# JoeMWatson/input-inference-for-control

Measured on AMD Instinct MI355X. Metric: i2c timestep-messages/sec (cell-iterations/s = B*T*EM-iters/s), pendulum T=200 B=4096 per GPU, higher is better.
Workload: dtype f64; 1 GPU; pendulum_known_quad cubature i2c (nx=2, nu=1, nz=4), T=200, B=4096 trajectories per GPU, global batch 4096, CubatureQuadrature(1,0,0), alpha0=100, tol=0; batch_per_gpu=4096, horizon=200, parallelism=batch-sharded x1, no collective in the EM loop, kernels=one lane per trajectory

## Files before the change

### input-inference-for-control_amd/csrc/i2c_cell.hpp

```cpp
#pragma once
#include <stdint.h>
#include <type_traits>
#include "../../include/i2c_hip.h"
#include "i2c_linalg.hpp"
#include "i2c_models.hpp"

namespace i2c {

template <typename R> struct Rule {
  R sf;
  R w0;
  R wi;
  R W;
  int unit;
  int gh_degree, gh_points;
  R gh_x[I2C_MAX_GH_DEGREE], gh_w[I2C_MAX_GH_DEGREE];
};

template <class M> struct PerTraj : M {};
template <class M> struct is_per_traj : std::false_type {};
template <class M> struct is_per_traj<PerTraj<M>> : std::true_type {};
template <typename R, bool PER_TRAJ> struct ParamsB {};
template <typename R> struct ParamsB<R, true> {
  const R* params_b;
// ... 524 lines not shown
inline thread_local GridLaneSim grid_lane_sim{0, nullptr};
inline void grid_sim_sync();
#endif
I2C_FN int grid_lane() {
#ifdef I2C_HOST_SIM
  return grid_lane_sim.l;
#else
  return (int)__builtin_amdgcn_mbcnt_hi(~0u, __builtin_amdgcn_mbcnt_lo(~0u, 0u));
#endif
}
template <int GRID> I2C_FN bool grid_writer() {
  if constexpr (GRID == GRID_WAVE) return grid_lane() == 0;
  else return true;
}
template <int GRID> I2C_FN void grid_read_before_write() {
#ifdef I2C_HOST_SIM
  if constexpr (GRID == GRID_WAVE) grid_sim_sync();
#endif
}
template <class M, int DIN, int DOUT, bool CROSS, typename R, class F>
I2C_FN void grid_transform_wave(const Rule<R>& rule, const R* m, const R* L, const F& f, R* my, R* Sy, R* Sxy);

template <int GRID, class M, class ST, int DIN, int DOUT, bool CROSS, bool UNITW = false, typename R, class F>
I2C_FN void transform(const Rule<R>& rule, const R* m, const R* Sin, const R* L, const F& f, R* my, R* Sy, R* Sxy,
                      const PolyTab<R>* tab = nullptr) {
  if constexpr (GRID == GRID_WAVE) {
    grid_transform_wave<M, DIN, DOUT, CROSS>(rule, m, L, f, my, Sy, Sxy);
  } else if constexpr (GRID != 0) {
    if constexpr (DIN <= 3) {
      if (rule.gh_degree == 3) return grid_transform_ct<M, 3, DIN, DOUT, CROSS>(rule, m, L, f, my, Sy, Sxy);
      if (rule.gh_degree == 4) return grid_transform_ct<M, 4, DIN, DOUT, CROSS>(rule, m, L, f, my, Sy, Sxy);
      if (rule.gh_degree == 2) return grid_transform_ct<M, 2, DIN, DOUT, CROSS>(rule, m, L, f, my, Sy, Sxy);
    }
    grid_transform<M, DIN, DOUT, CROSS>(rule, m, L, f, my, Sy, Sxy);
  } else
    sp_transform<M, ST, DIN, DOUT, CROSS, UNITW>(rule, m, Sin, L, f, my, Sy, Sxy, tab);
}


template <typename R, typename S = R> struct FwdArgs {
  const S* prior;
  S* fwd;
  S* prior_out;
  const R* x0;
  const R* sig_x0;
  const R* z;
  const R* alpha;
  const R* alpha_cell;
  const uint8_t* ff;
  int32_t* status;
  const uint8_t* expert;
};

template <class M, typename R, bool LEAN = false, int GRID = 0, typename ST_ = R>
I2C_HD inline void forward_sweep_body(const Consts<M, R>& c, const FwdArgs<R, ST_>& a, const int b) {
  using C = Consts<M, R>;
  constexpr int NX = C::NX, NU = C::NU, NZ = C::NZ, NZT = C::NZT, D = C::D;
  constexpr unsigned W = sizeof(ST_);
  const unsigned long B = c.B;
  const int T = c.T;
  const unsigned bo = (unsigned)b * W;
  const unsigned rb0 = (unsigned)(B * W);
  const R alpha_traj = a.alpha[b];
  const bool wr = grid_writer<GRID>();
  int fail = 0;

  R mu_x[NX], sig_x[sym(NX)];
#pragma unroll
  for (int i = 0; i < NX; ++i) mu_x[i] = a.x0[i * B + b];
#pragma unroll
  for (int i = 0; i < sym(NX); ++i) sig_x[i] = a.sig_x0[i * B + b];

  constexpr bool VOFF = C::D <= 5;
  unsigned voff[VOFF ? C::E_FWD : 1];
  if (VOFF) {
#pragma unroll
    for (int e = 0; e < C::E_FWD; ++e) voff[e] = bo + (unsigned)e * rb0;
  }
  constexpr bool PREFETCH = C::D <= 5;
  R pri[C::E_PRI], zt[NZ];
  if (PREFETCH) {
    const unsigned rb = rb0;
    const Window w = make_window(a.prior + (unsigned long)(LEAN ? 0 : c.row(0)) * C::E_POST * B, (unsigned long)C::E_POST * rb);
#pragma unroll
    for (int e = 0; e < C::E_PRI; ++e) pri[e] = (R)wld<ST_>(w, VOFF ? 0u : (e) * rb, VOFF ? voff[e] : bo);
#pragma unroll
    for (int k = 0; k < NZ; ++k) zt[k] = (!LEAN && c.z_per_cell) ? a.z[((long)c.row(0) * NZ + k) * B + b] : c.zg[k];
  }

  unsigned ff_cur = a.ff[LEAN ? 0 : c.row(0)];
  constexpr bool STRUCT_L0 = C::D <= 5;
  R Lx[STRUCT_L0 ? sym(NX) : 1];
  if (STRUCT_L0) {
    R rx[NX];
#pragma unroll
    for (int i = 0; i < sym(NX); ++i) Lx[i] = sig_x[i];
    fail = note_failure(fail, chol<NX>(Lx, rx), 1, 0);
  }

  ff_cur = opaque(ff_cur);
  if (PREFETCH) {
#pragma unroll
    for (int e = 0; e < C::E_PRI; ++e) pri[e] = opaque(pri[e]);
#pragma unroll
    for (int k = 0; k < NZ; ++k) zt[k] = opaque(zt[k]);
  }
#pragma unroll
  for (int i = 0; i < NX; ++i) mu_x[i] = opaque(mu_x[i]);
#pragma unroll
  for (int i = 0; i < sym(NX); ++i) sig_x[i] = opaque(sig_x[i]);
  const R alpha_settled = opaque(alpha_traj);
  R alpha_cur = opaque((!LEAN && a.alpha_cell) ? a.alpha_cell[(long)c.row(0) * B + b] : alpha_settled);
  constexpr bool CONST_V = VOFF && (sym(NZ) + sym(NX) <= 16);
  PolyTab<R> ptab;
  if (CONST_V) poly_tab_init(ptab);
  const PolyTab<R>* const tab = CONST_V ? &ptab : nullptr;
  R xi0_v[CONST_V ? sym(NZ) : 1], eta_v[CONST_V ? sym(NX) : 1];
  if (CONST_V) {
#pragma unroll
    for (int i = 0; i < sym(NZ); ++i) xi0_v[i] = opaque(c.sig_xi0[i]);
#pragma unroll
    for (int i = 0; i < sym(NX); ++i) eta_v[i] = opaque(LEAN ? c.sig_eta[i] : c.sig_eta_w[i]);
  }

  for (int t = 0; t < T; ++t) {
    const int tn = t + 1 < T ? t + 1 : t;
    const int tr = LEAN ? t : c.row(t), tnr = LEAN ? tn : c.row(tn);
    const unsigned rb = opaque_uniform(rb0);
    const int kz = (C::D >= 6) ? (int)opaque_uniform(0u) : 0;
    if (!PREFETCH) {
      const Window w = make_window(a.prior + (unsigned long)tr * C::E_POST * B, (unsigned long)C::E_POST * rb);
#pragma unroll
      for (int e = 0; e < C::E_PRI; ++e) pri[e] = (R)wld<ST_>(w, VOFF ? 0u : (e) * rb, VOFF ? voff[e] : bo);
#pragma unroll
      for (int k = 0; k < NZ; ++k) zt[k] = (!LEAN && c.z_per_cell) ? a.z[((long)tr * NZ + k) * B + b] : c.zg[k];
    }

    const R alpha = opaque(alpha_cur);
    const R* pmu = pri;
    const R* psig = pri + D;
    const R* Kprev = pri + D + sym(D);

    int cell_bad = 0;
    R mu0[D], S0[sym(D)];
    R L0[STRUCT_L0 ? sym(D) : 1], Luu[sym(NU)], ruu[NU];
    if (ff_cur != 0) {
#pragma unroll
      for (int i = 0; i < NX; ++i) mu0[i] = mu_x[i];
#pragma unroll
      for (int i = NX; i < D; ++i) mu0[i] = pmu[i];
#pragma unroll
      for (int i = 0; i < D; ++i)
#pragma unroll
        for (int j = 0; j <= i; ++j)
          S0[tri(i, j)] = (i < NX) ? sig_x[tri(i, j)] : (j >= NX ? psig[tri(i, j)] : R(0));
      if (STRUCT_L0) {
#pragma unroll
        for (int p = 0; p < NU; ++p)
#pragma unroll
          for (int q = 0; q <= p; ++q) Luu[tri(p, q)] = psig[tri(NX + p, NX + q)];
#pragma unroll
        for (int p = 0; p < NU; ++p)
#pragma unroll
          for (int j = 0; j < NX; ++j) L0[tri(NX + p, j)] = R(0);
      }
    } else {
      R S[sym(NX)], delta[NX];
#pragma unroll
      for (int i = 0; i < sym(NX); ++i) S[i] = psig[i] + sig_x[i];
#pragma unroll
      for (int i = 0; i < NX; ++i) delta[i] = mu_x[i] - pmu[i];
      bool ok;
      const R rho = pdf_ratio<NX>(S, delta, &ok, tab);
      cell_bad = flag_stage(cell_bad, ok, 0);
      R Kt[NU * NX];
#pragma unroll
      for (int i = 0; i < NU * NX; ++i) Kt[i] = rho * Kprev[i];
// ... 59 lines not shown
      R mz[NZ], Sz[sym(NZ)], Sxz[D * NZ];
      transform<GRID, M, ObsStruct<M>, D, NZ, true, LEAN>(c.rule_xu, mu0, S0, L, ObserveF<M, R>{params_of(c, b)}, mz, Sz, Sxz, tab);
#pragma unroll
      for (int i = 0; i < sym(NZ); ++i) Sz[i] += alpha * (CONST_V ? xi0_v[i] : c.sig_xi0[i + kz]);
      cell_bad = flag_stage(cell_bad, kalman_update<D, NZ>(mu0, S0, mz, Sz, Sxz, zt), 2);
    }
    if (!LEAN && PREFETCH && c.z_per_cell) {
#pragma unroll
      for (int k = 0; k < NZ; ++k) zt[k] = a.z[((long)tnr * NZ + k) * B + b];
    }
    const Window out = make_window(a.fwd + (unsigned long)t * C::E_FWD * B, (unsigned long)C::E_FWD * rb);
    if (wr) {
#pragma unroll
      for (int e = 0; e < D; ++e) wst(out, VOFF ? 0u : (e) * rb, VOFF ? voff[e] : bo, (ST_)mu0[e]);
#pragma unroll
      for (int e = 0; e < sym(D); ++e) wst(out, VOFF ? 0u : (D + e) * rb, VOFF ? voff[D + e] : bo, (ST_)S0[e]);
    }

    sched_fence<(D >= 6)>();
    R Sxy[D * NX];
    {
      R L[sym(D)], rinv[D];
#pragma unroll
      for (int i = 0; i < sym(D); ++i) L[i] = S0[i];
      cell_bad = flag_stage(cell_bad, chol<D>(L, rinv), 3);
      transform<GRID, M, DenseStruct<D>, D, NX, true, LEAN>(c.rule_xu, mu0, S0, L, DynamicsF<M, R>{params_of(c, b)}, mu_x, sig_x, Sxy, tab);
    }
#pragma unroll
    for (int i = 0; i < sym(NX); ++i) sig_x[i] += CONST_V ? eta_v[i] : (LEAN ? c.sig_eta[i + kz] : c.sig_eta_w[i + kz]);
    R L3[sym(NX)], rinv3[NX];
#pragma unroll
    for (int i = 0; i < sym(NX); ++i) L3[i] = sig_x[i];
    cell_bad = flag_stage(cell_bad, chol<NX>(L3, rinv3), 4);
    sched_fence<(D >= 6)>();
#pragma unroll
    for (int i = 0; i < D; ++i) {
      fsub<NX>(L3, rinv3, &Sxy[i * NX]);
      bsub<NX>(L3, rinv3, &Sxy[i * NX]);
      sched_fence<(D >= 6)>();
    }

    ff_cur = opaque(ff_cur);
    if (!LEAN) {
      alpha_cur = opaque(alpha_cur);
      if (PREFETCH) {
#pragma unroll
        for (int k = 0; k < NZ; ++k) zt[k] = opaque(zt[k]);
      }
    }
    if (PREFETCH) {
#pragma unroll
      for (int e = 0; e < C::E_PRI; ++e) pri[e] = opaque(pri[e]);
    }
    if (wr) {
#pragma unroll
      for (int e = 0; e < D * NX; ++e) wst(out, VOFF ? 0u : (D + sym(D) + NX + sym(NX) + e) * rb, VOFF ? voff[D + sym(D) + NX + sym(NX) + e] : bo, (ST_)Sxy[e]);
    }
    sched_fence<(D >= 6)>();

    if (NZT > 0 && t == c.terminal_cell && c.has_Qf) {
      constexpr int NT = C::NZT1;
      R mzt[NT], Szt[sym(NT)], Sxzt[NX * NT];
      transform<GRID, M, TermStruct<M>, NX, NT, true, LEAN>(c.rule_x, mu_x, sig_x, L3, ObserveTermF<M, R>{params_of(c, b)}, mzt, Szt, Sxzt);
#pragma unroll
      for (int i = 0; i < sym(NT); ++i) Szt[i] += alpha * c.sig_xiT0[i];
      cell_bad = flag_stage(cell_bad, kalman_update<NX, NT>(mu_x, sig_x, mzt, Szt, Sxzt, c.zg_term), 5);
      if (STRUCT_L0) {
#pragma unroll
        for (int i = 0; i < sym(NX); ++i) L3[i] = sig_x[i];
        cell_bad = flag_stage(cell_bad, chol<NX>(L3, rinv3), 5);
      }
    }
    if (STRUCT_L0) {
#pragma unroll
      for (int i = 0; i < sym(NX); ++i) Lx[i] = L3[i];
    }
    fail = fold_cell_failure(fail, cell_bad, t);
    if (wr) {
#pragma unroll
      for (int e = 0; e < NX; ++e) wst(out, VOFF ? 0u : (D + sym(D) + e) * rb, VOFF ? voff[D + sym(D) + e] : bo, (ST_)mu_x[e]);
#pragma unroll
      for (int e = 0; e < sym(NX); ++e) wst(out, VOFF ? 0u : (D + sym(D) + NX + e) * rb, VOFF ? voff[D + sym(D) + NX + e] : bo, (ST_)sig_x[e]);
    }

  }
  if (wr && fail != 0 && a.status[b] == 0) a.status[b] = fail;
}


template <class M, typename R, int GRID = 0>
I2C_FN void end_of_chain(const Consts<M, R>& c, R* temp, const int b, const R* m3f, const R* S3f, R* m3m, R* S3m,
                         int32_t* status) {
  constexpr int NX = M::NX;
  const bool wr = grid_writer<GRID>();
  if (c.has_x_terminal) {
    const R tmp = temp[b];
    grid_read_before_write<GRID>();
    if (wr) temp[b] = tmp + c.dtemp;
    R St[sym(NX)], Ssum[sym(NX)], rinv[NX];
#pragma unroll
    for (int i = 0; i < sym(NX); ++i) {
      St[i] = tmp * S3f[i];
      Ssum[i] = c.sig_x_term[i] + St[i];
    }
    bool ok = chol<NX>(Ssum, rinv);
    R Wm[NX * NX];
#pragma unroll
    for (int j = 0; j < NX; ++j) {
      R col[NX];
#pragma unroll
      for (int i = 0; i < NX; ++i) col[i] = St[tri_any(i, j)];
      fsub<NX>(Ssum, rinv, col);
#pragma unroll
      for (int i = 0; i < NX; ++i) Wm[i * NX + j] = col[i];
    }
#pragma unroll
    for (int i = 0; i < NX; ++i)
#pragma unroll
      for (int j = 0; j <= i; ++j) {
        R v = St[tri(i, j)];
#pragma unroll
        for (int k = 0; k < NX; ++k) v -= Wm[k * NX + i] * Wm[k * NX + j];
        S3m[tri(i, j)] = v;
      }
    R r1[NX], r2[NX], Lt[sym(NX)], LT[sym(NX)];
#pragma unroll
    for (int i = 0; i < sym(NX); ++i) {
      Lt[i] = St[i];
      LT[i] = c.sig_x_term[i];
    }
    ok = chol<NX>(Lt, rinv) && ok;
#pragma unroll
    for (int i = 0; i < NX; ++i) r1[i] = m3f[i];
    fsub<NX>(Lt, rinv, r1);
    bsub<NX>(Lt, rinv, r1);
    ok = chol<NX>(LT, rinv) && ok;
#pragma unroll
    for (int i = 0; i < NX; ++i) r2[i] = c.mu_x_term[i];
// ... 1229 lines not shown
```

### input-inference-for-control_amd/csrc/i2c_impl.hpp

```cpp
#pragma once
#include "i2c_entry.hpp"
#include "i2c_cell.hpp"
#include "i2c_group.hpp"
#include "i2c_wave.hpp"
#include "i2c_quad.hpp"
#include "i2c_grid.hpp"
#include "i2c_linearize.hpp"

#include <cmath>
#include <cstdlib>
#include <cstring>

namespace i2c {

constexpr int SWEEP_BLOCK = 64;
#ifndef I2C_LANE_BLOCK
#define I2C_LANE_BLOCK 64
#endif
constexpr int LANE_BLOCK = I2C_LANE_BLOCK;
constexpr int CELL_BLOCK = 256;

#ifdef I2C_HOST_SIM
#define I2C_KERNEL(BLOCK) static void
#define I2C_LANE_PARAMS const long lane_x_, const int lane_y_,
#define I2C_LANE_X(BLOCK) ((void)lane_y_, lane_x_)
#define I2C_LANE_Y lane_y_
template <class K, class... A>
static int launch(K kernel, const long n, const int ny, const int , void* , const A&... args) {
  for (int y = 0; y < ny; ++y)
    for (long x = 0; x < n; ++x) kernel(x, y, args...);
  return I2C_OK;
}
static int copy_bytes(void* dst, const void* src, size_t n, void*) {
  std::memcpy(dst, src, n);
  return I2C_OK;
}
#else
#define I2C_KERNEL(BLOCK) __global__ __launch_bounds__(BLOCK) void
#define I2C_LANE_PARAMS
#define I2C_LANE_X(BLOCK) ((long)blockIdx.x * (BLOCK) + threadIdx.x)
#define I2C_LANE_Y ((int)blockIdx.y)
static int sweep_lanes() {
  static int v = [] {
    const char* e = getenv("I2C_SWEEP_LANES");
    const int n = e ? atoi(e) : LANE_BLOCK;
    return (n >= 1 && n <= LANE_BLOCK) ? n : LANE_BLOCK;
  }();
  return v;
}
template <class K, class... A>
static int launch(K kernel, const long n, const int ny, const int block, void* stream, const A&... args) {
  hipLaunchKernelGGL(kernel, dim3((unsigned)((n + block - 1) / block), ny), dim3(block), 0, (hipStream_t)stream, args...);
  return hipGetLastError() == hipSuccess ? I2C_OK : I2C_ELAUNCH;
}
static int copy_bytes(void* dst, const void* src, size_t n, void* stream) {
  return hipMemcpyAsync(dst, src, n, hipMemcpyDeviceToDevice, (hipStream_t)stream) == hipSuccess ? I2C_OK : I2C_ELAUNCH;
}
#endif

template <class M, typename R, bool LEAN, bool GRID = false, typename S = R>
I2C_KERNEL(LANE_BLOCK) k_forward(I2C_LANE_PARAMS const Consts<M, R> c, const FwdArgs<R, S> a, const int block) {
  const long b = I2C_LANE_X(block);
// ... 163 lines not shown

template <typename R> struct PendingMstep {
  const R* part;
  R* term_stats;
  MstepArgs<R> ms;
  int n_chunks;
  R tol;
};
template <class M, typename R> I2C_FN void finish_pending_mstep(const Consts<M, R>& c, const PendingMstep<R>& pm, const int b) {
  using C = Consts<M, R>;
  constexpr int P = REDUCE_PARTS;
  const long B = c.B;
  const int nc = pm.n_chunks;
  const R alpha = pm.ms.alpha[b];
  const R trT = (C::NZT > 0 && c.has_Qf) ? pm.term_stats[b] : R(0);
  R sm[P], sv[P];
#pragma unroll
  for (int q = 0; q < P; ++q) sm[q] = sv[q] = R(0);
  for (int t0 = 0; t0 < nc; t0 += 2 * P) {
    R pm_t[2 * P], pv_t[2 * P];
#pragma unroll
    for (int i = 0; i < 2 * P; ++i) {
      const long t = t0 + i < nc ? t0 + i : nc - 1;
      pm_t[i] = pm.part[(t * 2 + 0) * B + b];
      pv_t[i] = pm.part[(t * 2 + 1) * B + b];
    }
#pragma unroll
    for (int i = 0; i < 2 * P; ++i) {
      const bool in = t0 + i < nc;
      sm[i % P] += in ? pm_t[i] : R(0);
      sv[i % P] += in ? pv_t[i] : R(0);
    }
  }
  R m = R(0), v = R(0);
#pragma unroll
  for (int q = 0; q < P; ++q) {
    m += sm[q];
    v += sv[q];
  }
  pm.term_stats[B + b] = m;
  pm.term_stats[2 * B + b] = v;
  Consts<M, R> cm = c;
  cm.tol = pm.tol;
  mstep_update<M, R>(cm, pm.ms, b, trT, m, v, m, alpha);
}
template <class M, typename R, bool LEAN, typename S = R>
I2C_KERNEL(LANE_BLOCK) k_forward_mstep(I2C_LANE_PARAMS const Consts<M, R> c, const FwdArgs<R, S> a, const int block, const PendingMstep<R> pm) {
  const long b = I2C_LANE_X(block);
  if (b < c.B) {
    finish_pending_mstep<M, R>(c, pm, (int)b);
    forward_sweep_body<M, R, LEAN, 0, S>(c, a, (int)b);
  }
}


template <typename R> static bool unit_rule(const Rule<R>& r) { return r.unit && r.w0 == R(0); }
template <class M, typename R> static bool unit_rule(const Consts<M, R>& c) { return unit_rule(c.rule_xu) && unit_rule(c.rule_x); }

#ifdef I2C_HOST_SIM
template <typename R, class Body>
static void sim_teams(const int team, const long n_teams, const int n_rows, const bool rows_on_team, const size_t lds, const Body& body) {
  for (int y0 = 0; y0 < (rows_on_team ? 1 : n_rows); ++y0)
    for (long i = 0; i < n_teams; ++i) {
      std::vector<R> sh(lds, R(0)), xch(128, R(0));
      HostBarrier bar(team);
      std::vector<std::thread> lanes;
      for (int l = 0; l < team; ++l)
        lanes.emplace_back([&, l] {
          for (int y = y0; y < (rows_on_team ? n_rows : y0 + 1); ++y) body(i, y, l, lds ? sh.data() : (R*)nullptr, &bar, xch.data());
        });
      for (auto& th : lanes) th.join();
    }
}
#else
template <class M, typename R> __device__ __forceinline__ const Consts<M, R>* kernarg_consts() {
  return (const Consts<M, R>*)__builtin_amdgcn_kernarg_segment_ptr();
}
template <class M, typename R> __device__ __forceinline__ const R* kernarg_zeta() {
  constexpr size_t zoff = (sizeof(Consts<M, R>) + alignof(ZetaArg<M, R>) - 1) / alignof(ZetaArg<M, R>) * alignof(ZetaArg<M, R>);
  return ((const ZetaArg<M, R>*)((const char*)__builtin_amdgcn_kernarg_segment_ptr() + zoff))->v;
}
__device__ __forceinline__ long xcd_first_traj(const unsigned i) {
  const unsigned x = i & 7u, r = (i >> 3) & 3u, g = i >> 5;
  return 16L * (g * 8u + x) + 4 * r;
}
static unsigned xcd_blocks(const long B) { return (unsigned)((B + 127) / 128) * 32u; }
#endif

enum { GK_FORWARD = 0, GK_BACKWARD = 1, GK_PROPAGATE = 2, GK_CKF = 3 };
template <int KIND, class M, typename R, int G, bool FULLW, class KC, class A>
I2C_FN void group_body(const Consts<M, R>& c, const KC& kc, const A& a, const int b, const Grp<R, G>& g) {
  if constexpr (KIND == GK_FORWARD) forward_group_body<M, R, G, FULLW>(c, kc, a, b, g);
  if constexpr (KIND == GK_BACKWARD) backward_group_body<M, R, G, FULLW>(c, kc, a, b, g);
  if constexpr (KIND == GK_PROPAGATE) propagate_group_body<M, R, G, FULLW>(c, kc, a, b, g);
  if constexpr (KIND == GK_CKF) ckf_group_body<M, R, G>(c, kc, a, b, g);
}
#ifndef I2C_HOST_SIM
template <int KIND, class M, typename R, int G, bool FULLW, class A>
__global__ __launch_bounds__(SWEEP_BLOCK) void k_group(const Consts<M, R> c, const ZetaArg<M, R> zeta, const int has_zeta, const A a) {
  __shared__ GConst<M, R> kc;
  __shared__ R sh[(SWEEP_BLOCK / G) * Grp<R, G>::SIZE];
  gconst_fill<M, R>(kc, kernarg_consts<M, R>(), has_zeta ? kernarg_zeta<M, R>() : (const R*)nullptr, (int)threadIdx.x, SWEEP_BLOCK);
  __syncthreads();
  const long lane = (long)blockIdx.x * SWEEP_BLOCK + threadIdx.x;
  const long b = lane / G;
  if (b >= c.B) return;
// ... 387 lines not shown
  c.t0 = p->t0;
  c.has_Qf = p->has_Qf && M::NZT > 0;
  c.has_x_terminal = p->has_x_terminal;
  c.z_per_cell = p->z_per_cell && p->z != nullptr;
  c.use_expert = use_expert;
  c.terminal_cell = p->terminal_cell;
  c.inference = p->inference;
  c.post_tm = (p->post_layout == 1 && M::WAVE) ? 1 : 0;
  auto is_diag = [](const double* W, int n) {
    for (int i = 0; i < n; ++i)
      for (int j = 0; j < i; ++j)
        if (W[i * (i + 1) / 2 + j] != 0.0) return 0;
    return 1;
  };
  c.qr_diag = is_diag(p->QR, C::NZ);
  c.qf_diag = is_diag(p->Qf, C::NZT);
  c.rule_xu = make_rule<R>(p, C::D);
  c.rule_x = make_rule<R>(p, C::NX);
  c.dtemp = (R)p->dtemp;
  c.tol = (R)tol;
  for (int i = 0; i < sym(C::NX); ++i) c.sig_eta[i] = (R)p->sig_eta[i];
  for (int i = 0; i < sym(C::NX); ++i) c.sig_eta_w[i] = c.rule_xu.W * c.sig_eta[i];
  for (int i = 0; i < sym(C::NZ); ++i) c.sig_xi0[i] = (R)p->sig_xi0[i];
  for (int i = 0; i < sym(C::NZ); ++i) c.QR[i] = (R)p->QR[i];
  for (int i = 0; i < sym(C::NZT); ++i) c.sig_xiT0[i] = (R)p->sig_xiT0[i];
  for (int i = 0; i < sym(C::NZT); ++i) c.Qf[i] = (R)p->Qf[i];
  for (int i = 0; i < C::NZ; ++i) c.zg[i] = (R)p->zg[i];
  for (int i = 0; i < C::NZT; ++i) c.zg_term[i] = (R)p->zg_term[i];
  for (int i = 0; i < C::NX; ++i) c.mu_x_term[i] = (R)p->mu_x_term[i];
  for (int i = 0; i < sym(C::NX); ++i) c.sig_x_term[i] = (R)p->sig_x_term[i];
  for (int i = 0; i < M::NP; ++i) c.params[i] = (R)p->model_params[i];
  if constexpr (is_per_traj<M>::value) c.params_b = (const R*)p->model_params_b;
  return c;
}

static void chunk_geometry(int B, int T, int* n_chunks, int* chunk_len) {
  static const int forced = [] {
    const char* e = getenv("I2C_CHUNKS");
    return e ? atoi(e) : 0;
  }();
  int nc = (65536 + B - 1) / B;
  if (nc > 32) nc = 32;
  if (nc > T / 4) nc = T / 4;
  if (forced > 0) nc = forced < T ? forced : T;
  if (nc < 1) nc = 1;
  const int len = (T + nc - 1) / nc;
  *chunk_len = len;
  *n_chunks = (T + len - 1) / len;
}
static bool chunk_four_passes() {
  const char* e = getenv("I2C_CHUNK_PASSES");
  return e && atoi(e) == 4;
}
template <class M> struct ChunkWork {
  size_t bnd, part, total;
  ChunkWork(const int B, const int n_chunks) {
    constexpr int NX = M::NX;
    const size_t n = (size_t)n_chunks * (size_t)B;
    bnd = n * (NX + NX * NX + sym(NX));
    part = bnd + n * (NX + sym(NX));
    total = part + n * 3;
  }
};
template <class M> static size_t workspace_elems(int B, int T) {
  int nc, len;
  chunk_geometry(B, T, &nc, &len);
  return ChunkWork<M>(B, nc).total;
}
template <class M, typename R, typename S> static ChunkArgs<R, S> chunk_args(const I2cProblem* p, const CellArgs<R, S>& a) {
  ChunkArgs<R, S> ch{a, (R*)p->work, nullptr, nullptr, 0, 0};
  chunk_geometry(p->B, p->T, &ch.n_chunks, &ch.chunk_len);
  const ChunkWork<M> w(p->B, ch.n_chunks);
  ch.bnd = ch.comp + w.bnd;
  ch.part = ch.comp + w.part;
  return ch;
}

#define I2C_MODEL_CONST(name, MEMBER, DEFAULT)                                                                      \
  template <class M, class = void> struct name : std::integral_constant<int, (DEFAULT)> {};                         \
  template <class M> struct name<M, std::void_t<decltype(M::MEMBER)>> : std::integral_constant<int, M::MEMBER> {};
I2C_MODEL_CONST(bwd_fused_min_b, BWD_FUSED_MIN_B, I2C_BWD_FUSED_MIN_B)
I2C_MODEL_CONST(quad_backward_min_b, QUAD_BACKWARD8_MIN_B, 0)
I2C_MODEL_CONST(quad_backward_max_b, QUAD_BACKWARD8_MAX_B, -1)
I2C_MODEL_CONST(quad_chunk_walk_min_b, QUAD_CHUNK_WALK_MIN_B, 0)
I2C_MODEL_CONST(quad_chunk_walk_max_b, QUAD_CHUNK_WALK_MAX_B, -1)
I2C_MODEL_CONST(quad_chunk_passes_min_b, QUAD_CHUNK_PASSES_MIN_B, 0)
I2C_MODEL_CONST(quad_chunk_passes_max_b, QUAD_CHUNK_PASSES_MAX_B, -1)
I2C_MODEL_CONST(quad_chunk_stitch_max_b, QUAD_CHUNK_STITCH_MAX_B, -1)
#undef I2C_MODEL_CONST


struct Plan {
  int forward, backward, propagate, filter;
  int schedule;
  int walker;
  int compose, stitch;
  int rule;
  bool fwd_tm;
  bool fusable;
};

template <class M, typename R, typename S = R> struct Impl {
  using C = Consts<M, R>;
  static constexpr bool MIXED = sizeof(S) != sizeof(R);
  static constexpr int G = M::GROUP;
  static constexpr bool HAS_GROUP = G > 0 && sizeof(R) == 8 && !MIXED;
  static constexpr bool LANE = !M::GROUP_ONLY;
  static constexpr bool HAS_WAVE = M::WAVE && sizeof(R) == 8;
  static constexpr bool HAS_QUAD = M::QUAD && sizeof(R) == 8;
  static constexpr bool WIDE = QG<M>::WIDE;
  static constexpr bool HAS_QUAD_BACKWARD = HAS_QUAD && quad_backward_exists<M>();
  static constexpr bool QUAD8 = HAS_QUAD_BACKWARD && !WIDE && LANE;
  static constexpr bool HAS_QUAD_CKF = HAS_QUAD && !MIXED && quad_ckf_exists<M>();
  static constexpr bool HAS_QUAD_PROP = HAS_QUAD && !MIXED && quad_propagate_exists<M>();
  static constexpr bool HAS_GRID = LANE && sizeof(R) == 8 && !MIXED;

  enum Request {
    REQ_DEFAULT,
    REQ_ONE_LANE,
    REQ_GROUP,
    REQ_WAVE,
    REQ_QUAD,
    REQ_QUAD_FORWARD,
    REQ_GRID,
    REQ_NOT_OURS
  };
  static Request request(const int lanes, const int inference) {
    if (lanes == 0) return REQ_DEFAULT;
    if (lanes == -1) return REQ_ONE_LANE;
    if (lanes == 64 && HAS_GRID && inference == I2C_INF_GAUSS_HERMITE) return REQ_GRID;
    if (lanes == 64 && (M::WAVE || M::QUAD)) return HAS_WAVE ? REQ_WAVE : (HAS_QUAD ? REQ_QUAD : REQ_DEFAULT);
    if (lanes == I2C_LANES_QUAD) return HAS_QUAD ? (WIDE ? REQ_QUAD : REQ_QUAD_FORWARD) : REQ_DEFAULT;
    return (HAS_GROUP && lanes == G) ? REQ_GROUP : REQ_NOT_OURS;
  }
// ... 169 lines not shown

  static Plan resolve(const I2cProblem* p) {
    const Rule<R> rule_xu = make_rule<R>(p, C::D), rule_x = make_rule<R>(p, C::NX);
    const bool unit_xu = unit_rule(rule_xu), unit = unit_xu && unit_rule(rule_x);
    const Request req = request(p->group_lanes, p->inference);
    Plan pl;
    pl.rule = p->inference;
    pl.forward = forward_family(p, req, unit);
    pl.backward = backward_family(p, req, unit);
    pl.propagate = propagate_family(p, req, unit_xu || p->inference == I2C_INF_LINEARIZE);
    pl.filter = filter_family(p, req == REQ_GRID ? request(p->group_lanes, I2C_INF_CUBATURE) : req);
    pl.schedule = backward_schedule(p, req, pl.backward);
    const bool chunked = pl.schedule == I2C_BWD_CHUNKED;
    pl.walker = chunked ? pl.backward : I2C_ENOTSUP;
    pl.compose = pl.stitch = pl.schedule < 0 ? pl.schedule : I2C_ENOTSUP;
    if (chunked && p->inference == I2C_INF_CUBATURE) {
      pl.compose = quad_compose(p, req, unit) ? I2C_FAMILY_QUAD : I2C_FAMILY_LANE;
      pl.stitch = (pl.compose == I2C_FAMILY_QUAD || quad_stitch_alone(p, req, unit)) ? I2C_FAMILY_QUAD : I2C_FAMILY_LANE;
    }
    pl.fwd_tm = !MIXED && pl.forward == I2C_FAMILY_QUAD && ((M::WAVE && pl.backward == I2C_FAMILY_WAVE) || (HAS_QUAD_BACKWARD && pl.backward == I2C_FAMILY_QUAD));
    pl.fusable = LANE && C::D <= 5 && p->inference == I2C_INF_CUBATURE && pl.forward == I2C_FAMILY_LANE && pl.propagate == I2C_FAMILY_LANE &&
                 rule_xu.unit && rule_x.unit && !(p->z_per_cell && p->z) && !p->alpha_cell && p->t0 == 0;
    return pl;
  }
  static int plan(const I2cProblem* p) { return resolve(p).schedule; }
  static int family_of(const I2cProblem* p, const int sweep) {
    const Plan pl = resolve(p);
    const int of_sweep[] = {pl.forward, pl.backward, pl.propagate, pl.filter, pl.compose, pl.stitch};
    return of_sweep[sweep];
  }
  static int schedule_with(const Plan& pl, const bool workspace) {
    if (pl.schedule != I2C_BWD_CHUNKED || workspace) return pl.schedule;
    return (pl.rule == I2C_INF_CUBATURE && pl.walker != I2C_FAMILY_QUAD) ? I2C_BWD_TWO_PASS : I2C_BWD_FUSED;
  }

  static I2cProblem with_unit_rule(const I2cProblem* p) {
    I2cProblem q = *p;
    q.quad_alpha = 1.0, q.quad_beta = 0.0, q.quad_kappa = 0.0;
    return q;
  }
  static C forward_consts(const I2cProblem* p) { return make_consts<M, R>(p, 0.0, p->inference == I2C_INF_LINEARIZE ? p->expert_controller : 0); }
  static C propagate_consts(const I2cProblem* p, const int use_expert) {
    if (p->inference != I2C_INF_LINEARIZE) return make_consts<M, R>(p, 0.0, use_expert);
    const I2cProblem q = with_unit_rule(p);
    return make_consts<M, R>(&q, 0.0, use_expert);
  }
  static C filter_consts(const I2cProblem* p) {
    I2cProblem q = with_unit_rule(p);
    q.inference = I2C_INF_CUBATURE;
    return make_consts<M, R>(&q, 0.0, 0);
  }

  static int run_forward(const I2cProblem* p, const Plan& pl, const C& c, const void* prior, void* fwd, void* prior_out, int32_t* status,
                         void* stream, const PendingMstep<R>* pend = nullptr) {
    if (pl.forward < 0) return pl.forward;
    if (pend && !defers_mstep(pl)) return I2C_EINVAL;
    const FwdArgs<R, S> a{(const S*)prior, (S*)fwd, (S*)prior_out, (const R*)p->x0, (const R*)p->sig_x0,
                          (const R*)p->z,  (const R*)p->alpha, (const R*)p->alpha_cell, p->feedforward, status, p->expert};
    if (pl.forward == I2C_FAMILY_WAVE) {
      if constexpr (HAS_WAVE) return launch_wave<WK_FORWARD, M, R, S>(c, a, stream);
    }
    if (pl.forward == I2C_FAMILY_QUAD) {
      if constexpr (HAS_QUAD) {
        C cq = c;
        cq.fwd_tm = pl.fwd_tm;
        return launch_quad_forward<M, R, S>(cq, a, stream);
      }
    }
    if (pl.forward == I2C_FAMILY_GROUP) {
      if constexpr (HAS_GROUP) return launch_group<GK_FORWARD, M, R, G>(c, nullptr, a, stream);
    }
    if (pl.forward == I2C_FAMILY_GRID) {
      if constexpr (HAS_GRID) return launch_grid<GRK_FORWARD, M, R>(c, a, stream);
    }
    if constexpr (LANE) {
      if constexpr (!MIXED) {
        if (pl.rule == I2C_INF_LINEARIZE) return launch(k_forward_lin<M, R>, p->B, 1, LANE_BLOCK, stream, c, a);
        if (pl.rule == I2C_INF_GAUSS_HERMITE) return launch(k_forward<M, R, false, true>, p->B, 1, LANE_BLOCK, stream, c, a, LANE_BLOCK);
      }
#ifdef I2C_HOST_SIM
      const int lanes = LANE_BLOCK;
#else
      const int lanes = sweep_lanes();
#endif
      const bool lean = c.rule_xu.unit && c.rule_x.unit && !c.z_per_cell && !a.alpha_cell && !a.prior_out && c.t0 == 0;
      if constexpr (SELF_STITCH) {
        if (pend) return lean ? launch(k_forward_mstep<M, R, true, S>, p->B, 1, lanes, stream, c, a, lanes, *pend)
                              : launch(k_forward_mstep<M, R, false, S>, p->B, 1, lanes, stream, c, a, lanes, *pend);
      }
      if (lean) return launch(k_forward<M, R, true, false, S>, p->B, 1, lanes, stream, c, a, lanes);
      return launch(k_forward<M, R, false, false, S>, p->B, 1, lanes, stream, c, a, lanes);
    }
    return I2C_ENOTSUP;
  }
  static int forward(const I2cProblem* p, const void* prior, void* fwd, void* prior_out, int32_t* status, void* stream) {
    return run_forward(p, resolve(p), forward_consts(p), prior, fwd, prior_out, status, stream);
  }

  struct MstepFuse {
    double tol;
    int update;
    void* stats_out;
    bool done;
    bool defer;
    bool deferred;
    PendingMstep<R> pending;
  };
  static constexpr bool SELF_STITCH = LANE && C::D <= 5;
  static bool self_stitches(const Plan& pl, const C& c) {
    return SELF_STITCH && pl.rule == I2C_INF_CUBATURE && pl.stitch == I2C_FAMILY_LANE && pl.walker == I2C_FAMILY_LANE && !c.has_x_terminal &&
           !chunk_four_passes();
  }
  static bool defers_mstep(const Plan& pl) { return SELF_STITCH && pl.rule == I2C_INF_CUBATURE && pl.forward == I2C_FAMILY_LANE; }
  static const R* terminal_alpha(const I2cProblem* p, const C& c) {
    return p->alpha_cell ? (const R*)p->alpha_cell + (long)c.row(p->T - 1) * (long)p->B : (const R*)p->alpha;
  }
  static int run_backward(const I2cProblem* p, const Plan& pl, const C& c, const void* fwd, void* xm, void* post, void* zpost, void* cell_stats,
                          void* term_stats, int32_t* status, void* stream, MstepFuse* fuse) {
    if (pl.backward < 0) return pl.backward;
    if (pl.schedule < 0) return pl.schedule;
    const MstepArgs<R> ms{(const R*)term_stats, fuse ? (R*)p->alpha : nullptr, fuse ? (R*)fuse->stats_out : nullptr, fuse ? fuse->update : 0};
    const CellArgs<R, S> a{(const S*)fwd,  (const S*)xm,   (const R*)p->z, (S*)post, (S*)zpost,
                           (R*)cell_stats, (R*)term_stats, (R*)p->temp,    status,   terminal_alpha(p, c)};
    const int mode = schedule_with(pl, p->work != nullptr);
    int rc = I2C_ENOTSUP;
    if (pl.backward == I2C_FAMILY_WAVE) {
      if constexpr (HAS_WAVE) {
        if (mode != I2C_BWD_TWO_PASS || !a.xm || !a.cell_stats) return launch_wave<WK_BACKWARD, M, R, S>(c, a, stream);
        rc = launch_wave<WK_SCAN, M, R, S>(c, a, stream);
        if (rc == I2C_OK) rc = launch_wave<WK_CELL, M, R, S>(c, a, stream);
        if (rc == I2C_OK) rc = launch_reduce<M, R>(c, a, ms, p->T, stream);
        if (fuse) fuse->done = true;
      }
      return rc;
    }
    if (pl.backward == I2C_FAMILY_QUAD) {
      if constexpr (HAS_QUAD_BACKWARD) {
        if constexpr (QUAD8) {
          if (mode == I2C_BWD_CHUNKED) return backward_chunked(p, pl, c, a, ms, fuse, stream);
        }
        return launch_quad_backward<M, R, S>(c, a, stream);
      }
    }
    if (pl.backward == I2C_FAMILY_GROUP) {
      if constexpr (HAS_GROUP) return launch_group<GK_BACKWARD, M, R, G>(c, nullptr, a, stream);
    }
    if (pl.backward == I2C_FAMILY_GRID) {
      if constexpr (HAS_GRID) return launch_grid<GRK_BACKWARD, M, R>(c, a, stream);
    }
    if constexpr (LANE) {
      if (mode == I2C_BWD_CHUNKED) return backward_chunked(p, pl, c, a, ms, fuse, stream);
      if (mode == I2C_BWD_FUSED) {
        if constexpr (!MIXED) {
          if (pl.rule == I2C_INF_LINEARIZE) return launch(k_bwd_lin<M, R>, p->B, 1, LANE_BLOCK, stream, c, a);
          if (pl.rule == I2C_INF_GAUSS_HERMITE) return launch(k_bwd_fused<M, R, true>, p->B, 1, LANE_BLOCK, stream, c, a);
        }
        const bool lean = I2C_WALK_LEAN && !a.xm && !a.zpost && !a.cell_stats && !c.z_per_cell;
        return lean ? launch(k_bwd_fused<M, R, false, S, true>, p->B, 1, LANE_BLOCK, stream, c, a)
                    : launch(k_bwd_fused<M, R, false, S>, p->B, 1, LANE_BLOCK, stream, c, a);
      }
      if (!a.xm || !a.cell_stats) return I2C_EINVAL;
      const ScanArgs<R, S> sc{a.fwd, const_cast<S*>(a.xm), (R*)p->temp, a.status};
      rc = launch(k_scan<M, R, S>, p->B, 1, LANE_BLOCK, stream, c, sc);
      if (rc == I2C_OK) rc = launch(k_cell<M, R, S>, p->B, p->T, CELL_BLOCK, stream, c, a);
      if (rc == I2C_OK) rc = launch_reduce<M, R>(c, a, ms, p->T, stream);
      if (fuse) fuse->done = true;
    }
    return rc;
  }
  static int backward_chunked(const I2cProblem* p, const Plan& pl, const C& c, const CellArgs<R, S>& a, const MstepArgs<R>& ms, MstepFuse* fuse,
                              void* stream) {
    int rc = I2C_ENOTSUP;
    if constexpr (LANE) {
      const ChunkArgs<R, S> ch = chunk_args<M>(p, a);
      const long B = p->B;
      const int nc = ch.n_chunks;
      const bool lin = !MIXED && pl.rule == I2C_INF_LINEARIZE, gh = !MIXED && pl.rule == I2C_INF_GAUSS_HERMITE;
      const bool self = self_stitches(pl, c);
      if (fuse) fuse->done = true;
      if (pl.compose == I2C_FAMILY_QUAD) {
        if constexpr (QUAD8) rc = launch_quad_chunk_compose<M, R, S>(c, ch, stream);
      } else {
        rc = launch(k_chunk_compose<M, R, S>, B, nc, LANE_BLOCK, stream, c, ch);
      }
      if (rc != I2C_OK) return rc;
      rc = I2C_ENOTSUP;
      if (pl.stitch == I2C_FAMILY_QUAD) {
        if constexpr (QUAD8) rc = launch_quad_chunk_stitch<M, R, S>(c, ch, stream);
      } else if (lin || gh) {
        if constexpr (!MIXED)
          rc = lin ? launch(k_chunk_stitch_lin<M, R>, B, 1, LANE_BLOCK, stream, c, ch) : launch(k_chunk_stitch<M, R, R, true>, B, 1, LANE_BLOCK, stream, c, ch);
      } else if (!self) {
        rc = launch(k_chunk_stitch<M, R, S>, B, 1, LANE_BLOCK, stream, c, ch);
      } else {
        rc = I2C_OK;
      }
      if (rc != I2C_OK) return rc;
      rc = I2C_ENOTSUP;
      if (pl.walker == I2C_FAMILY_QUAD) {
        if constexpr (QUAD8) rc = launch_quad_chunk_walk<M, R, S>(c, ch, stream);
      } else if (lin || gh) {
        if constexpr (!MIXED)
          rc = lin ? launch(k_chunk_walk_lin<M, R>, B, nc, LANE_BLOCK, stream, c, ch) : launch(k_chunk_walk<M, R, R, false, true>, B, nc, LANE_BLOCK, stream, c, ch);
      } else {
        const bool lean = I2C_WALK_LEAN && !a.xm && !a.zpost && !a.cell_stats && !c.z_per_cell;
        if constexpr (SELF_STITCH) {
          if (self)
            rc = lean ? launch(k_chunk_walk_self<M, R, S, true>, B, nc, LANE_BLOCK, stream, c, ch)
                      : launch(k_chunk_walk_self<M, R, S>, B, nc, LANE_BLOCK, stream, c, ch);
        }
        if (!self) rc = lean ? launch(k_chunk_walk<M, R, S, true>, B, nc, LANE_BLOCK, stream, c, ch) : launch(k_chunk_walk<M, R, S>, B, nc, LANE_BLOCK, stream, c, ch);
      }
      if (rc != I2C_OK) return rc;
      if (lin) {
        if constexpr (!MIXED) rc = launch(k_chunk_reduce_lin<M, R>, B, 1, LANE_BLOCK, stream, c, ch, ms);
      } else if (self && fuse && fuse->defer) {
        fuse->deferred = true;
        fuse->pending = PendingMstep<R>{ch.part, a.term_stats, ms, nc, c.tol};
      } else {
        C cr = c;
        cr.T = nc;
        CellArgs<R, S> ared = a;
        ared.cell_stats = ch.part;
        rc = launch_reduce<M, R>(cr, ared, ms, p->T, stream);
      }
    }
    return rc;
  }
  static int backward(const I2cProblem* p, const void* fwd, void* xm, void* post, void* zpost, void* cell_stats,
                      void* term_stats, int32_t* status, void* stream) {
    return run_backward(p, resolve(p), make_consts<M, R>(p, 0.0, 0), fwd, xm, post, zpost, cell_stats, term_stats, status, stream, nullptr);
  }

  static int riccati(const I2cProblem* p, const void* prior_out, const void* fwd, const void* xm, void* post, void* ric,
                     int32_t* status, void* stream) {
    if constexpr (MIXED) return I2C_ENOTSUP;
    if constexpr (LANE) {
      if (!lane_request(p->group_lanes)) return I2C_ENOTSUP;
      const C c = make_consts<M, R>(p, 0.0, 0);
      RiccatiArgs<R> a{(const R*)prior_out, (const R*)fwd, (const R*)xm, (const R*)p->z, (const R*)p->alpha,
                       (R*)post,            (R*)ric,       status};
      return launch(k_riccati<M, R>, p->B, 1, LANE_BLOCK, stream, c, a);
    }
    return I2C_ENOTSUP;
  }

  static int run_mstep(const I2cProblem* p, const C& c, const void* term_stats, int update, void* stats_out, void* stream) {
    MstepArgs<R> a{(const R*)term_stats, (R*)p->alpha, (R*)stats_out, update};
    return launch(k_mstep<M, R>, p->B, 1, LANE_BLOCK, stream, c, a);
  }
  static int mstep(const I2cProblem* p, const void* term_stats, double tol, int update, void* stats_out, void* stream) {
    return run_mstep(p, make_consts<M, R>(p, tol, 0), term_stats, update, stats_out, stream);
  }

  static int to_feedback(const I2cProblem* p, int tau, void* stream) {
    const int n = tau + 1 < p->T ? tau + 1 : p->T;
    return launch(k_to_feedback<M>, n, 1, CELL_BLOCK, stream, const_cast<uint8_t*>(p->feedforward), p->t0, n, p->T);
  }

  static int learn(const I2cProblem* p, void* post, void* fwd, void* xm, void* zpost, void* cell_stats,
                   void* term_stats, double tol, int tau, int n_iters, void* stats_hist, int32_t* status,
                   void* stream) {
    const Plan pl = resolve(p);
    const C cf = forward_consts(p), cb = make_consts<M, R>(p, tol, 0);
    PendingMstep<R> pend{};
    bool have_pend = false;
    for (int it = 0; it < n_iters; ++it) {
      void* stats = (R*)stats_hist + (size_t)it * 4 * p->B;
      MstepFuse fuse{tol, 1, stats, false, it + 1 < n_iters && defers_mstep(pl), false, {}};
      int rc = run_forward(p, pl, cf, post, fwd, nullptr, status, stream, have_pend ? &pend : nullptr);
      have_pend = false;
      if (rc == I2C_OK) rc = run_backward(p, pl, cb, fwd, xm, post, zpost, cell_stats, term_stats, status, stream, &fuse);
      if (rc == I2C_OK && fuse.deferred) pend = fuse.pending, have_pend = true;
      if (rc == I2C_OK && !fuse.done) rc = run_mstep(p, cb, term_stats, 1, stats, stream);
      if (rc == I2C_OK && tau > 0 && it == 0) rc = to_feedback(p, tau, stream);
      if (rc != I2C_OK) return rc;
    }
    return I2C_OK;
  }

  static int learn_propagate(const I2cProblem* p, void* post, void* fwd, void* xm, void* zpost, void* cell_stats, void* term_stats,
                             void* prop, void* prop_hist, double tol, int tau, int n_iters, void* stats_hist, int use_expert,
                             int overlap, int32_t* status, void* stream) {
    if constexpr (MIXED) return I2C_ENOTSUP;
    const Plan pl = resolve(p);
    const C cf = forward_consts(p), cb = make_consts<M, R>(p, tol, 0), cp = propagate_consts(p, use_expert);
    auto prop_row = [&](int it) { return (void*)((R*)prop_hist + (size_t)it * 3 * p->B); };
    int pending = -1;
    for (int it = 0; it < n_iters; ++it) {
      int rc = I2C_OK;
      bool fused = false;
      if constexpr (LANE && C::D <= 5) {
        if (overlap && pl.fusable && pending >= 0) {
          FwdArgs<R> af{(const R*)post, (R*)fwd, nullptr, (const R*)p->x0, (const R*)p->sig_x0, (const R*)p->z, (const R*)p->alpha,
                        (const R*)p->alpha_cell, p->feedforward, status, p->expert};
          PropArgs<R> ap{(const R*)post, (R*)prop, (R*)prop_row(pending), (const R*)p->x0, (const R*)p->sig_x0,
                         (const R*)p->z, p->feedforward, status, p->expert};
          rc = launch(k_forward_propagate<M, R, true>, p->B, 2, LANE_BLOCK, stream, cp, af, ap);
          fused = true;
          pending = -1;
        }
      }
      if (!fused) {
        if (pending >= 0) {
          rc = run_propagate(p, pl, cp, post, prop, prop_row(pending), status, stream);
          pending = -1;
          if (rc != I2C_OK) return rc;
        }
        rc = run_forward(p, pl, cf, post, fwd, nullptr, status, stream);
      }
      if (rc != I2C_OK) return rc;
      void* stats = (R*)stats_hist + (size_t)it * 4 * p->B;
      MstepFuse fuse{tol, 1, stats, false};
      rc = run_backward(p, pl, cb, fwd, xm, post, zpost, cell_stats, term_stats, status, stream, &fuse);
      if (rc != I2C_OK) return rc;
      if (it == 0) {
        rc = run_propagate(p, pl, cp, post, prop, prop_row(0), status, stream);
        if (rc != I2C_OK) return rc;
      } else {
        pending = it;
      }
      if (!fuse.done) rc = run_mstep(p, cb, term_stats, 1, stats, stream);
      if (rc == I2C_OK && tau > 0 && it == 0) rc = to_feedback(p, tau, stream);
// ... 141 lines not shown
```

Before: 2.376 billion timestep-messages/s.

## Overlap chunk composition with forward sweep via helper wave in same workgroup

Adds a forward kernel variant that launches two waves per block. One wave runs the forward sweep and signals with workgroup barriers each time a chunk of timesteps is written. The second wave waits on those barriers and composes each finished chunk, so the backward pass can skip its separate compose launch. This hides compose latency behind the serial forward sweep, at the cost of doubling threads per block, adding barrier synchronisation, and relying on hand-written inline asm for the conditional barrier.

```diff
diff --git a/input-inference-for-control_amd/csrc/i2c_cell.hpp b/input-inference-for-control_amd/csrc/i2c_cell.hpp
--- a/input-inference-for-control_amd/csrc/i2c_cell.hpp
+++ b/input-inference-for-control_amd/csrc/i2c_cell.hpp
@@ -600,8 +600,36 @@
   const uint8_t* expert;
 };
 
-template <class M, typename R, bool LEAN = false, int GRID = 0, typename ST_ = R>
-I2C_HD inline void forward_sweep_body(const Consts<M, R>& c, const FwdArgs<R, ST_>& a, const int b) {
+struct NoRelease {
+  static constexpr bool ON = false;
+  int chunk_len;
+  I2C_HD inline void release() const {}
+  I2C_HD inline void release_if(int, int) const {}
+};
+struct ChunkRelease {
+  static constexpr bool ON = true;
+  int chunk_len;
+  I2C_HD inline void release() const {
+#if defined(__HIP_DEVICE_COMPILE__)
+    __builtin_amdgcn_fence(__ATOMIC_RELEASE, "workgroup");
+    __builtin_amdgcn_s_waitcnt(0x0F70);
+    __builtin_amdgcn_s_barrier();
+#endif
+  }
+  I2C_HD inline void release_if(const int t, const int at) const {
+#if defined(__HIP_DEVICE_COMPILE__)
+    asm volatile("s_cmp_lg_u32 %0, %1\n\ts_cbranch_scc1 .Lnot_released_%=\n\ts_waitcnt vmcnt(0)\n\ts_barrier\n.Lnot_released_%=:"
+                 :
+                 : "s"(t), "s"(at)
+                 : "memory", "scc");
+#else
+    (void)t, (void)at;
+#endif
+  }
+};
+
+template <class M, typename R, bool LEAN = false, int GRID = 0, typename ST_ = R, class REL = NoRelease>
+I2C_HD inline void forward_sweep_body(const Consts<M, R>& c, const FwdArgs<R, ST_>& a, const int b, const REL rel = REL{0}) {
   using C = Consts<M, R>;
   constexpr int NX = C::NX, NU = C::NU, NZ = C::NZ, NZT = C::NZT, D = C::D;
   constexpr unsigned W = sizeof(ST_);
@@ -671,6 +699,7 @@
     for (int i = 0; i < sym(NX); ++i) eta_v[i] = opaque(LEAN ? c.sig_eta[i] : c.sig_eta_w[i]);
   }
 
+  [[maybe_unused]] int next_release = rel.chunk_len;
   for (int t = 0; t < T; ++t) {
     const int tn = t + 1 < T ? t + 1 : t;
     const int tr = LEAN ? t : c.row(t), tnr = LEAN ? tn : c.row(tn);
@@ -836,6 +865,10 @@
 #pragma unroll
       for (int e = 0; e < C::E_PRI; ++e) pri[e] = opaque(pri[e]);
     }
+    if constexpr (REL::ON) {
+      rel.release_if(t, next_release);
+      next_release += t == next_release ? rel.chunk_len : 0;
+    }
     if (wr) {
 #pragma unroll
       for (int e = 0; e < D * NX; ++e) wst(out, VOFF ? 0u : (D + sym(D) + NX + sym(NX) + e) * rb, VOFF ? voff[D + sym(D) + NX + sym(NX) + e] : bo, (ST_)Sxy[e]);
@@ -868,6 +901,7 @@
     }
 
   }
+  if constexpr (REL::ON) rel.release();
   if (wr && fail != 0 && a.status[b] == 0) a.status[b] = fail;
 }
 
diff --git a/input-inference-for-control_amd/csrc/i2c_impl.hpp b/input-inference-for-control_amd/csrc/i2c_impl.hpp
--- a/input-inference-for-control_amd/csrc/i2c_impl.hpp
+++ b/input-inference-for-control_amd/csrc/i2c_impl.hpp
@@ -8,6 +8,7 @@
 #include "i2c_linearize.hpp"
 
 #include <cmath>
+#include <cstdio>
 #include <cstdlib>
 #include <cstring>
 
@@ -277,6 +278,45 @@
     forward_sweep_body<M, R, LEAN, 0, S>(c, a, (int)b);
   }
 }
+
+template <class M, typename R, bool LEAN, typename S, bool MSTEP>
+I2C_FN void forward_helper_lane(const Consts<M, R>& c, const FwdArgs<R, S>& a, const ChunkArgs<R, S>& ch, const PendingMstep<R>& pm,
+                                const int role, const int b) {
+  if (role == 0) {
+    if constexpr (MSTEP) finish_pending_mstep<M, R>(c, pm, b);
+    forward_sweep_body<M, R, LEAN, 0, S, ChunkRelease>(c, a, b, ChunkRelease{ch.chunk_len});
+  } else {
+    for (int k = 0; k < ch.n_chunks; ++k) {
+#if defined(__HIP_DEVICE_COMPILE__)
+      __builtin_amdgcn_s_barrier();
+      __builtin_amdgcn_fence(__ATOMIC_ACQUIRE, "workgroup");
+#endif
+      chunk_compose_body<M, R, S>(c, ch, k, b);
+    }
+  }
+}
+#ifdef I2C_HOST_SIM
+constexpr int HELPER_WAVES = 1;
+#define I2C_HELPER_LANES                                                                \
+  const long b = I2C_LANE_X(LANE_BLOCK);                                                \
+  for (int role = 0; role < 2; ++role)
+#else
+constexpr int HELPER_WAVES = 2;
+#define I2C_HELPER_LANES                                                                \
+  const long b = (long)blockIdx.x * LANE_BLOCK + (threadIdx.x & (LANE_BLOCK - 1));      \
+  const int role = __builtin_amdgcn_readfirstlane((int)(threadIdx.x / LANE_BLOCK));     \
+  if (b < c.B)
+#endif
+template <class M, typename R, bool LEAN, typename S = R>
+I2C_KERNEL(2 * LANE_BLOCK) k_forward_helper(I2C_LANE_PARAMS const Consts<M, R> c, const FwdArgs<R, S> a, const ChunkArgs<R, S> ch) {
+  I2C_HELPER_LANES forward_helper_lane<M, R, LEAN, S, false>(c, a, ch, PendingMstep<R>{}, role, (int)b);
+}
+template <class M, typename R, bool LEAN, typename S = R>
+I2C_KERNEL(2 * LANE_BLOCK) k_forward_mstep_helper(I2C_LANE_PARAMS const Consts<M, R> c, const FwdArgs<R, S> a, const ChunkArgs<R, S> ch,
+                                                  const PendingMstep<R> pm) {
+  I2C_HELPER_LANES forward_helper_lane<M, R, LEAN, S, true>(c, a, ch, pm, role, (int)b);
+}
+#undef I2C_HELPER_LANES
 
 
 template <typename R> static bool unit_rule(const Rule<R>& r) { return r.unit && r.w0 == R(0); }
@@ -770,6 +810,10 @@
   const char* e = getenv("I2C_CHUNK_PASSES");
   return e && atoi(e) == 4;
 }
+static bool plan_trace() {
+  const char* e = getenv("I2C_TRACE_PLAN");
+  return e && atoi(e) == 1;
+}
 template <class M> struct ChunkWork {
   size_t bnd, part, total;
   ChunkWork(const int B, const int n_chunks) {
@@ -798,6 +842,7 @@
   template <class M, class = void> struct name : std::integral_constant<int, (DEFAULT)> {};                         \
   template <class M> struct name<M, std::void_t<decltype(M::MEMBER)>> : std::integral_constant<int, M::MEMBER> {};
 I2C_MODEL_CONST(bwd_fused_min_b, BWD_FUSED_MIN_B, I2C_BWD_FUSED_MIN_B)
+I2C_MODEL_CONST(forward_helper_min_b, FORWARD_HELPER_MIN_B, 4096)
 I2C_MODEL_CONST(quad_backward_min_b, QUAD_BACKWARD8_MIN_B, 0)
 I2C_MODEL_CONST(quad_backward_max_b, QUAD_BACKWARD8_MAX_B, -1)
 I2C_MODEL_CONST(quad_chunk_walk_min_b, QUAD_CHUNK_WALK_MIN_B, 0)
@@ -1073,7 +1118,7 @@
   }
 
   static int run_forward(const I2cProblem* p, const Plan& pl, const C& c, const void* prior, void* fwd, void* prior_out, int32_t* status,
-                         void* stream, const PendingMstep<R>* pend = nullptr) {
+                         void* stream, const PendingMstep<R>* pend = nullptr, const ChunkArgs<R, S>* helper = nullptr) {
     if (pl.forward < 0) return pl.forward;
     if (pend && !defers_mstep(pl)) return I2C_EINVAL;
     const FwdArgs<R, S> a{(const S*)prior, (S*)fwd, (S*)prior_out, (const R*)p->x0, (const R*)p->sig_x0,
@@ -1105,6 +1150,16 @@
       const int lanes = sweep_lanes();
 #endif
       const bool lean = c.rule_xu.unit && c.rule_x.unit && !c.z_per_cell && !a.alpha_cell && !a.prior_out && c.t0 == 0;
+      if (plan_trace()) fprintf(stderr, "i2c_forward_lane: sweep=%s\n", SELF_STITCH && helper ? "helper" : "plain");
+      if constexpr (SELF_STITCH) {
+        if (helper) {
+          constexpr int W = HELPER_WAVES;
+          if (pend) return lean ? launch(k_forward_mstep_helper<M, R, true, S>, W * (long)p->B, 1, W * LANE_BLOCK, stream, c, a, *helper, *pend)
+                                : launch(k_forward_mstep_helper<M, R, false, S>, W * (long)p->B, 1, W * LANE_BLOCK, stream, c, a, *helper, *pend);
+          return lean ? launch(k_forward_helper<M, R, true, S>, W * (long)p->B, 1, W * LANE_BLOCK, stream, c, a, *helper)
+                      : launch(k_forward_helper<M, R, false, S>, W * (long)p->B, 1, W * LANE_BLOCK, stream, c, a, *helper);
+        }
+      }
       if constexpr (SELF_STITCH) {
         if (pend) return lean ? launch(k_forward_mstep<M, R, true, S>, p->B, 1, lanes, stream, c, a, lanes, *pend)
                               : launch(k_forward_mstep<M, R, false, S>, p->B, 1, lanes, stream, c, a, lanes, *pend);
@@ -1126,7 +1181,23 @@
     bool defer;
     bool deferred;
     PendingMstep<R> pending;
+    bool composed;
   };
+  static int forward_helper_knob() {
+    const char* e = getenv("I2C_FORWARD_HELPER");
+    if (chunk_four_passes() || (e && strcmp(e, "0") == 0)) return 0;
+    return e ? 1 : -1;
+  }
+  static bool forward_helper_on(const I2cProblem* p, const Plan& pl, const C& c) {
+#ifndef I2C_HOST_SIM
+    if (sweep_lanes() != LANE_BLOCK) return false;
+#endif
+    const int knob = forward_helper_knob();
+    if (knob == 0 || (knob < 0 && p->B < forward_helper_min_b<M>::value)) return false;
+    const bool to_chunked = pl.backward == I2C_FAMILY_LANE || (QUAD8 && pl.backward == I2C_FAMILY_QUAD);
+    return SELF_STITCH && LANE_BLOCK == 64 && pl.forward == I2C_FAMILY_LANE && pl.rule == I2C_INF_CUBATURE && to_chunked &&
+           schedule_with(pl, p->work != nullptr) == I2C_BWD_CHUNKED && pl.compose == I2C_FAMILY_LANE && !c.has_x_terminal;
+  }
   static constexpr bool SELF_STITCH = LANE && C::D <= 5;
   static bool self_stitches(const Plan& pl, const C& c) {
     return SELF_STITCH && pl.rule == I2C_INF_CUBATURE && pl.stitch == I2C_FAMILY_LANE && pl.walker == I2C_FAMILY_LANE && !c.has_x_terminal &&
@@ -1199,7 +1270,11 @@
       const bool lin = !MIXED && pl.rule == I2C_INF_LINEARIZE, gh = !MIXED && pl.rule == I2C_INF_GAUSS_HERMITE;
       const bool self = self_stitches(pl, c);
       if (fuse) fuse->done = true;
-      if (pl.compose == I2C_FAMILY_QUAD) {
+      const bool composed = fuse && fuse->composed;
+      if (plan_trace()) fprintf(stderr, "i2c_backward_chunked: compose=%s\n", composed ? "skipped" : "launched");
+      if (composed) {
+        rc = I2C_OK;
+      } else if (pl.compose == I2C_FAMILY_QUAD) {
         if constexpr (QUAD8) rc = launch_quad_chunk_compose<M, R, S>(c, ch, stream);
       } else {
         rc = launch(k_chunk_compose<M, R, S>, B, nc, LANE_BLOCK, stream, c, ch);
@@ -1286,10 +1361,14 @@
     const C cf = forward_consts(p), cb = make_consts<M, R>(p, tol, 0);
     PendingMstep<R> pend{};
     bool have_pend = false;
+    const bool helper = forward_helper_on(p, pl, cf);
+    CellArgs<R, S> of_fwd{};
+    of_fwd.fwd = (const S*)fwd;
+    const ChunkArgs<R, S> chunks = helper ? chunk_args<M>(p, of_fwd) : ChunkArgs<R, S>{};
     for (int it = 0; it < n_iters; ++it) {
       void* stats = (R*)stats_hist + (size_t)it * 4 * p->B;
-      MstepFuse fuse{tol, 1, stats, false, it + 1 < n_iters && defers_mstep(pl), false, {}};
-      int rc = run_forward(p, pl, cf, post, fwd, nullptr, status, stream, have_pend ? &pend : nullptr);
+      MstepFuse fuse{tol, 1, stats, false, it + 1 < n_iters && defers_mstep(pl), false, {}, helper};
+      int rc = run_forward(p, pl, cf, post, fwd, nullptr, status, stream, have_pend ? &pend : nullptr, helper ? &chunks : nullptr);
       have_pend = false;
       if (rc == I2C_OK) rc = run_backward(p, pl, cb, fwd, xm, post, zpost, cell_stats, term_stats, status, stream, &fuse);
       if (rc == I2C_OK && fuse.deferred) pend = fuse.pending, have_pend = true;
```

New measurement: 2.427 billion timestep-messages/s (median of 6 runs). +2.1%, better.
